# chernistry/sentio

Hardware: NVIDIA H100
Metric: retrieval queries/sec @1M docs,1024-d,top_k=100 (higher is better)
Workload: dtype f16 store / f32 scan / f64 exact re-score

## Files before the change

sentio_b200/csrc/dense_mma.cu:

```cuda
#include <cuda.h>

#include <math.h>

#include <algorithm>
#include <vector>

#include "dense_common.cuh"
#include "dense_mma.cuh"
#include "wgmma.cuh"

namespace {

constexpr int kTileRows = 128;
constexpr int kBK = 64;
constexpr uint32_t kATileBytes = kTileRows * kBK * 2;
constexpr int kConsumerWarps = 8;
constexpr int kMmaThreads = 32 * kConsumerWarps + 32;
constexpr int kQbnMax = 256;
constexpr int kSampleRows = 16;
constexpr int kSampleKeys = kTileRows / kSampleRows;
constexpr int kSelectThreads = 512;
constexpr int kSelStage = 8192;
constexpr int kSelTop = 2048;

__device__ __forceinline__ void tma_load_2d(uint32_t dst, const CUtensorMap* map, int c0, int c1, uint32_t bar,
                                            uint64_t policy) {
  asm volatile(
      "cp.async.bulk.tensor.2d.shared::cluster.global.mbarrier::complete_tx::bytes.L2::cache_hint [%0], [%1, {%2, %3}], "
      "[%4], %5;" ::"r"(dst),
      "l"(map), "r"(c0), "r"(c1), "r"(bar), "l"(policy)
      : "memory");
}
__device__ __forceinline__ void tma_prefetch_l2_2d(const CUtensorMap* map, int c0, int c1) {
  asm volatile("cp.async.bulk.prefetch.tensor.2d.L2.global [%0, {%1, %2}];" ::"l"(map), "r"(c0), "r"(c1) : "memory");
}

struct MmaScanParams {
  const float* inv_norm;
  const float* thr_init;
  unsigned long long* cand;
  int32_t* counts;
  int32_t* fallback;
  int64_t n;
  int32_t kb_count;
  int32_t num_tiles;
  int32_t tile_first, tile_step;
  int32_t capg;
  int32_t stages;
  int32_t prefetch;
  const uint32_t* mask;
  int32_t mask_qs;
  const float* hh;
  const float* rq;
};

template <int QBN, bool FILTER, bool EUCLID>
__global__ void __launch_bounds__(kMmaThreads, 1)
dense_scan_mma_kernel(const __grid_constant__ CUtensorMap tm_rows, const __grid_constant__ CUtensorMap tm_q,
                      const MmaScanParams p) {
  extern __shared__ uint8_t msm_raw[];
  const uint32_t raw = smem_u32(msm_raw);
  const uint32_t base = (raw + 1023u) & ~1023u;
  uint8_t* sm = msm_raw + (base - raw);
  constexpr uint32_t kQBoxBytes = QBN * kBK * 2;
  constexpr uint32_t kStageBytes = kATileBytes + kQBoxBytes;
  uint64_t* bars = reinterpret_cast<uint64_t*>(sm + (size_t)p.stages * kStageBytes);
  const uint32_t bar_full = smem_u32(bars), bar_empty = smem_u32(bars + p.stages);
  volatile float* thr = reinterpret_cast<volatile float*>(bars + 2 * p.stages);
  int* cnt = reinterpret_cast<int*>(const_cast<float*>(thr) + QBN);
  float* rq_s = reinterpret_cast<float*>(cnt + QBN);

  const int warp = threadIdx.x >> 5, lane = threadIdx.x & 31;
  const int grid = gridDim.x, cta = blockIdx.x;
  const int my_tiles = cta < p.num_tiles ? (p.num_tiles - 1 - cta) / grid + 1 : 0;
  auto tile_row = [&](int t) { return (p.tile_first + (cta + t * grid) * p.tile_step) * kTileRows; };

  if (threadIdx.x == 0) {
    for (int s = 0; s < p.stages; ++s) {
      mbar_init(bar_full + 8 * s, 1);
      mbar_init(bar_empty + 8 * s, kConsumerWarps);
    }
    mbar_fence_init();
    asm volatile("prefetch.tensormap [%0];" ::"l"(&tm_rows) : "memory");
    asm volatile("prefetch.tensormap [%0];" ::"l"(&tm_q) : "memory");
  }
  for (int i = threadIdx.x; i < QBN; i += blockDim.x) {
    thr[i] = p.thr_init ? p.thr_init[i] : -INFINITY;
    cnt[i] = 0;
    if constexpr (EUCLID) rq_s[i] = p.rq[i];
  }
  __syncthreads();

  if (warp == kConsumerWarps) {
    if (lane == 0) {
      const uint64_t pol_corpus = policy_evict_first();
      const uint64_t pol_query = policy_evict_last();
      int it = 0;
      const int total_it = my_tiles * p.kb_count;
      for (int t = 0; t < my_tiles; ++t) {
        const int row = tile_row(t);
        for (int kb = 0; kb < p.kb_count; ++kb, ++it) {
          const int s = it % p.stages;
          const uint32_t use = (uint32_t)(it / p.stages);
          const int pf = it + p.stages + p.prefetch;
          if (p.prefetch > 0 && pf < total_it) {
            const int pt = pf / p.kb_count, pkb = pf - pt * p.kb_count;
            tma_prefetch_l2_2d(&tm_rows, pkb * kBK, tile_row(pt));
          }
          if (it >= p.stages) mbar_wait(bar_empty + 8 * s, (use & 1u) ^ 1u);
          const uint32_t stage = base + (uint32_t)s * kStageBytes;
          mbar_expect_tx(bar_full + 8 * s, kStageBytes);
          tma_load_2d(stage, &tm_rows, kb * kBK, row, bar_full + 8 * s, pol_corpus);
          tma_load_2d(stage + kATileBytes, &tm_q, kb * kBK, 0, bar_full + 8 * s, pol_query);
        }
      }
    }
  } else {
    const int wg = warp >> 2;
    unsigned long long* my_cand = p.cand + (size_t)cta * p.capg;
    const size_t q_stride = (size_t)grid * p.capg;
    int it = 0;
    for (int t = 0; t < my_tiles; ++t) {
      float acc[QBN / 2];
      for (int kb = 0; kb < p.kb_count; ++kb, ++it) {
        const int s = it % p.stages;
        mbar_wait(bar_full + 8 * s, (uint32_t)(it / p.stages) & 1u);
        const uint32_t stage = base + (uint32_t)s * kStageBytes;
        const uint64_t da = wgmma_desc_sw128(stage + (uint32_t)wg * (kATileBytes / 2));
        const uint64_t db = wgmma_desc_sw128(stage + kATileBytes);
        wgmma_fence();
#pragma unroll
        for (int k = 0; k < kBK / 16; ++k)
          Wgmma<QBN>::mma(acc, da + (uint64_t)(2 * k), db + (uint64_t)(2 * k), (kb | k) ? 1u : 0u);
        wgmma_commit();
        wgmma_wait<1>();
        __syncwarp();
        if (kb > 0 && lane == 0) mbar_arrive(bar_empty + 8 * ((it - 1) % p.stages));
      }
      wgmma_wait<0>();
      __syncwarp();
      if (lane == 0) mbar_arrive(bar_empty + 8 * ((it - 1) % p.stages));
      const int64_t row0 = (int64_t)tile_row(t) + wg * 64 + (warp & 3) * 16 + (lane >> 2);
      const bool live0 = row0 < p.n, live1 = row0 + 8 < p.n;
      const float invn0 = live0 ? __ldg(p.inv_norm + row0) : 0.f;
      const float invn1 = live1 ? __ldg(p.inv_norm + row0 + 8) : 0.f;
      float h0 = 0.f, h1 = 0.f;
      if constexpr (EUCLID) {
        h0 = live0 ? __ldg(p.hh + row0) : 0.f;
        h1 = live1 ? __ldg(p.hh + row0 + 8) : 0.f;
      }
      auto key = [&](float a, float invn, float h, int col) {
        float s = a * invn;
        if constexpr (EUCLID) s = __fsub_rn(__fmul_rn(rq_s[col], s), h);
        return s;
      };
      const uint32_t* mrow = nullptr;
      if constexpr (FILTER) mrow = p.mask + (size_t)(row0 >> 5) * p.mask_qs + 2 * (lane & 3);
      const int sh0 = (int)(row0 & 31), sh1 = sh0 + 8;
      if (p.thr_init == nullptr) {
        const int slot = t * kSampleKeys + warp;
#pragma unroll
        for (int j = 0; j < QBN / 4; j += 2) {
          uint2 mw = make_uint2(0u, 0u);
          if constexpr (FILTER) mw = __ldg(reinterpret_cast<const uint2*>(mrow + 4 * j));
#pragma unroll
          for (int e = 0; e < 2; ++e) {
            bool m0 = live0, m1 = live1;
            if constexpr (FILTER) {
              const uint32_t w = e ? mw.y : mw.x;
              m0 = m0 && ((w >> sh0) & 1u);
              m1 = m1 && ((w >> sh1) & 1u);
            }
            const int col = 4 * j + 2 * (lane & 3) + e;
            const float s0 = m0 ? key(acc[2 * j + e], invn0, h0, col) : -INFINITY;
            const float s1 = m1 ? key(acc[2 * j + 2 + e], invn1, h1, col) : -INFINITY;
            uint32_t best = max(f32_orderable(s0), f32_orderable(s1));
            best = max(best, __shfl_xor_sync(0xffffffffu, best, 4));
            best = max(best, __shfl_xor_sync(0xffffffffu, best, 8));
            best = max(best, __shfl_xor_sync(0xffffffffu, best, 16));
            if (lane < 4) my_cand[(size_t)col * q_stride + slot] = ((unsigned long long)best << 32) | 0xffffffffull;
          }
        }
      } else {
#pragma unroll
        for (int j = 0; j < QBN / 4; j += 2) {
          uint2 mw = make_uint2(0u, 0u);
          if constexpr (FILTER) mw = __ldg(reinterpret_cast<const uint2*>(mrow + 4 * j));
#pragma unroll
          for (int h = 0; h < 2; ++h) {
            if (!(h ? live1 : live0)) continue;
            const int64_t row = row0 + 8 * h;
            const float invn = h ? invn1 : invn0;
            const float hrow = h ? h1 : h0;
#pragma unroll
            for (int e = 0; e < 2; ++e) {
              const int col = 4 * j + 2 * (lane & 3) + e;
              const float score = key(acc[2 * j + 2 * h + e], invn, hrow, col);
              bool match = true;
              if constexpr (FILTER) match = ((e ? mw.y : mw.x) >> (h ? sh1 : sh0)) & 1u;
              if (score >= thr[col] && match) {
                const int pos = atomicAdd(&cnt[col], 1);
                if (pos < p.capg) my_cand[(size_t)col * q_stride + pos] = make_key32(score, (uint32_t)row);
              }
            }
          }
        }
      }
    }
  }
  __syncthreads();
  for (int i = threadIdx.x; i < QBN; i += blockDim.x) {
    const int c = p.thr_init == nullptr ? my_tiles * kSampleKeys : cnt[i];
    p.counts[(size_t)i * grid + cta] = min(c, p.capg);
    if (c > p.capg && p.fallback) p.fallback[i] = 1;
  }
}

struct SelectParams {
  const unsigned long long* cand;
  const int32_t* counts;
  int32_t grid, capg;
  int32_t nq;
  int32_t mode;
  float* thr_out;
  const float* eps;
  int32_t* fallback;
  const __half* rows;
  const float* q;
  int32_t d_pad, ch;
  int64_t id_base;
  int32_t k;
  int64_t* out_ids;
  double* out_scores;
  int32_t* out_counts;
  const int32_t* state;
  int32_t metric;
  const double* cfac;
  const float* rows32;
};

template <bool FILTER, bool F32>
__global__ void __launch_bounds__(kSelectThreads, 2) dense_select_kernel(const SelectParams p) {
  extern __shared__ __align__(16) uint8_t ssm[];
  unsigned long long* keys = reinterpret_cast<unsigned long long*>(ssm);
  unsigned long long* top = keys + kSelStage;
  unsigned long long* ek = top + kSelTop;
  uint32_t* ei = reinterpret_cast<uint32_t*>(ek + kSelTop);
  __shared__ double qq_s;
  __shared__ int s_prefix[kSelectThreads + 1];
  __shared__ int s_hist[256];
  __shared__ int s_scal[4];
  __shared__ int s_ntop;
  const int tid = threadIdx.x, nt = blockDim.x, lane = tid & 31, warp = tid >> 5, nw = nt >> 5, qi = blockIdx.x;
  const int K = p.k, G = p.grid;
  if (p.mode == 0 && qi >= p.nq) {
    if (tid == 0) p.thr_out[qi] = INFINITY;
    return;
  }
  if constexpr (FILTER) {
    if (p.state[qi]) {
      if (p.mode == 0 && tid == 0) p.thr_out[qi] = INFINITY;
      return;
    }
  }
  if (p.fallback[qi] != 0) {
    if (p.mode == 0 && tid == 0) p.thr_out[qi] = INFINITY;
    return;
  }
  const int32_t* counts = p.counts + (size_t)qi * G;
  const unsigned long long* cand = p.cand + (size_t)qi * G * p.capg;
  {
    const int v = tid < G ? counts[tid] : 0;
    int x = v;
    for (int o = 1; o < 32; o <<= 1) {
      const int y = __shfl_up_sync(0xffffffffu, x, o);
      if (lane >= o) x += y;
    }
    if (lane == 31) s_hist[warp] = x;
    if (tid == 0) s_ntop = 0;
    __syncthreads();
    if (warp == 0) {
      int w = lane < nw ? s_hist[lane] : 0;
      for (int o = 1; o < 32; o <<= 1) {
        const int y = __shfl_up_sync(0xffffffffu, w, o);
        if (lane >= o) w += y;
      }
      s_hist[32 + lane] = w;
    }
    __syncthreads();
    const int incl = x + (warp ? s_hist[32 + warp - 1] : 0);
    if (tid < G) s_prefix[tid] = incl - v;
    if (tid == G - 1) s_prefix[G] = incl;
    __syncthreads();
  }
  const int total = s_prefix[G];
  const bool staged = total <= kSelStage;
  if (staged) {
    for (int g = warp; g < G; g += nw) {
      const int c = s_prefix[g + 1] - s_prefix[g];
      const unsigned long long* src = cand + (size_t)g * p.capg;
      unsigned long long* dst = keys + s_prefix[g];
      for (int i = lane; i < c; i += 32) dst[i] = src[i];
    }
    __syncthreads();
  }
#define SB_FOR_EACH_KEY(BODY)                                                       \
  if (staged) {                                                                     \
    for (int i_ = tid; i_ < total; i_ += nt) {                                      \
      const unsigned long long key = keys[i_];                                      \
      BODY                                                                          \
    }                                                                               \
  } else {                                                                          \
    for (int g_ = warp; g_ < G; g_ += nw) {                                         \
      const int c_ = s_prefix[g_ + 1] - s_prefix[g_];                               \
      const unsigned long long* src_ = cand + (size_t)g_ * p.capg;                  \
      for (int i_ = lane; i_ < c_; i_ += 32) {                                      \
        const unsigned long long key = src_[i_];                                    \
        BODY                                                                        \
      }                                                                             \
    }                                                                               \
  }

  unsigned long long prefix = 0ull, mask = 0ull;
  if (total > K) {
    int need = K;
    for (int shift = 56; shift >= 0; shift -= 8) {
      for (int i = tid; i < 256; i += nt) s_hist[i] = 0;
      __syncthreads();
      SB_FOR_EACH_KEY(if ((key & mask) == prefix) {
        const int dgt = (int)((key >> shift) & 0xffull);
        const unsigned grp = __match_any_sync(__activemask(), dgt);
        if ((int)(threadIdx.x & 31) == __ffs(grp) - 1) atomicAdd(&s_hist[dgt], __popc(grp));
      })
      __syncthreads();
      if (warp == 0) warp_select_bin<true>(s_hist, need, lane, s_scal);
      __syncthreads();
      prefix |= (unsigned long long)s_scal[0] << shift;
      mask |= 0xffull << shift;
      need = s_scal[1];
      const int bucket = s_scal[2];
      __syncthreads();
      if (bucket <= 16) break;
    }
  }
  const float eps = p.eps[qi];
  const unsigned long long lo_key = total > K ? window_lo_key(prefix, eps) : 0ull;
  if (p.mode == 0) {
    if (tid == 0) p.thr_out[qi] = total > K ? key32_score(lo_key) : -INFINITY;
    return;
  }
  SB_FOR_EACH_KEY(if (key >= lo_key) {
    const int at = atomicAdd(&s_ntop, 1);
    if (at < kSelTop) top[at] = key;
  })
#undef SB_FOR_EACH_KEY
  __syncthreads();
  const int ntop = s_ntop;
  if (ntop > kSelTop) {
    if (tid == 0) p.fallback[qi] = 1;
    return;
  }
  int P = 32;
  while (P < ntop) P <<= 1;
  RescoreArgs ra;
  ra.rows = p.rows;
  ra.q = p.q + (size_t)qi * p.d_pad;
  ra.d_pad = p.d_pad;
  ra.ch = p.ch;
  ra.id_base = p.id_base;
  ra.k = p.k;
  ra.out_ids = p.out_ids + (size_t)qi * p.k;
  ra.out_scores = p.out_scores + (size_t)qi * p.k;
  ra.out_count = p.out_counts + qi;
  ra.metric = p.metric;
  ra.cfac = p.cfac;
  ra.rows32 = p.rows32;
  rescore_and_emit<F32>(top, ntop, P, ek, ei, &qq_s, reinterpret_cast<float*>(keys), ra);
}

typedef CUresult (*EncodeTiledFn)(CUtensorMap*, CUtensorMapDataType, cuuint32_t, void*, const cuuint64_t*,
                                  const cuuint64_t*, const cuuint32_t*, const cuuint32_t*, CUtensorMapInterleave,
                                  CUtensorMapSwizzle, CUtensorMapL2promotion, CUtensorMapFloatOOBfill);

int encode_map(CUtensorMap* map, const void* ptr, int64_t rows, int64_t cols, int box_rows) {
  static EncodeTiledFn fn = nullptr;
  if (!fn) {
    void* pfn = nullptr;
    cudaDriverEntryPointQueryResult qres;
    if (cudaGetDriverEntryPoint("cuTensorMapEncodeTiled", &pfn, cudaEnableDefault, &qres) == cudaSuccess &&
        qres == cudaDriverEntryPointSuccess)
      fn = reinterpret_cast<EncodeTiledFn>(pfn);
  }
  SB_REQUIRE(fn != nullptr, SB_ERR_CUDA, "cuTensorMapEncodeTiled entry point not available");
  cuuint64_t dims[2] = {(cuuint64_t)cols, (cuuint64_t)rows};
  cuuint64_t strides[1] = {(cuuint64_t)cols * 2};
  cuuint32_t box[2] = {(cuuint32_t)kBK, (cuuint32_t)box_rows};
  cuuint32_t estr[2] = {1, 1};
  CUresult r = fn(map, CU_TENSOR_MAP_DATA_TYPE_FLOAT16, 2, const_cast<void*>(ptr), dims, strides, box, estr,
                  CU_TENSOR_MAP_INTERLEAVE_NONE, CU_TENSOR_MAP_SWIZZLE_128B, CU_TENSOR_MAP_L2_PROMOTION_L2_256B,
                  CU_TENSOR_MAP_FLOAT_OOB_FILL_NONE);
  SB_REQUIRE(r == CUDA_SUCCESS, SB_ERR_CUDA, "cuTensorMapEncodeTiled failed with CUresult %d", (int)r);
  return SB_OK;
}

size_t mma_per_query(bool euclid) { return euclid ? 12 : 8; }
int mma_stages(const sb_ctx* ctx, int qbn, bool euclid = false) {
  const size_t stage = kATileBytes + (size_t)qbn * kBK * 2 + 16;
  const size_t fixed = 1024 + (size_t)qbn * mma_per_query(euclid);
  return std::min((int)((ctx->smem_optin - fixed) / stage), ctx->dense_max_stages);
}
size_t mma_smem(int qbn, int stages, bool euclid) {
  return 1024 + (size_t)stages * (kATileBytes + (size_t)qbn * kBK * 2 + 16) + (size_t)qbn * mma_per_query(euclid);
}

template <int QBN, bool FILTER, bool EUCLID>
int launch_mma(const CUtensorMap& tm_rows, const CUtensorMap& tm_q, const MmaScanParams& mp, int grid, size_t smem,
               cudaStream_t st) {
  auto kern = dense_scan_mma_kernel<QBN, FILTER, EUCLID>;
  SB_CUDA(cudaFuncSetAttribute(kern, cudaFuncAttributeMaxDynamicSharedMemorySize, (int)smem));
  kern<<<grid, kMmaThreads, smem, st>>>(tm_rows, tm_q, mp);
  SB_CUDA(cudaGetLastError());
  return SB_OK;
}

template <bool FILTER, bool EUCLID>
int dispatch_mma(int qbn, const CUtensorMap& tm_rows, const CUtensorMap& tm_q, const MmaScanParams& mp, int grid,
                 size_t smem, cudaStream_t st) {
  switch (qbn) {
    case 16: return launch_mma<16, FILTER, EUCLID>(tm_rows, tm_q, mp, grid, smem, st);
    case 32: return launch_mma<32, FILTER, EUCLID>(tm_rows, tm_q, mp, grid, smem, st);
    case 64: return launch_mma<64, FILTER, EUCLID>(tm_rows, tm_q, mp, grid, smem, st);
    case 128: return launch_mma<128, FILTER, EUCLID>(tm_rows, tm_q, mp, grid, smem, st);
    case 256: return launch_mma<256, FILTER, EUCLID>(tm_rows, tm_q, mp, grid, smem, st);
  }
  sb_set_error("dense_mma: unsupported query block %d", qbn);
  return SB_ERR_UNSUPPORTED;
}

}

bool dense_mma_eligible(const sb_ctx* ctx, const DenseIndex& ix, int B) {
  if (B < 16) return false;
  if (ix.d_pad % kBK != 0 || ix.n_pad % kTileRows != 0) return false;
  if (ix.n < 64 * kTileRows) return false;
  return mma_stages(ctx, kQbnMax) >= 3;
}

int dense_mma_topk_enqueue(sb_ctx* ctx, DenseIndex& ix, const float* q_pad, int B, int k, int64_t* out_ids,
                           double* out_scores, int32_t* out_counts, cudaStream_t st, const DenseFilter* flt) {
  const int kb_count = ix.d_pad / kBK;
  const int total_tiles = (int)(ix.n_pad / kTileRows);
  const int gsz = kQbnMax;
  const int grid = std::min(ctx->num_sms, total_tiles);
  const double phi = flt ? std::min(1.0, (double)std::max<int64_t>(flt->c_min, 1) / (double)ix.n) : 1.0;
  const double hit = flt ? 1.0 - pow(1.0 - phi, (double)kSampleRows) : 1.0;
  const double m_eff = flt ? (double)kSampleRows * phi / hit : (double)kSampleRows;
  const int per_cta = flt ? std::max(ctx->dense_sample_per_cta,
                                     (int)ceil(4.0 * k / ((double)kSampleKeys * hit * grid)))
                          : std::max(ctx->dense_sample_per_cta, std::min(8, (4 * k / kSampleKeys + grid - 1) / grid));
  const int sample_tiles = (int)std::min<int64_t>((int64_t)per_cta * grid, total_tiles);
  const int sample_step = total_tiles / sample_tiles;
  const int sgrid = std::min(grid, sample_tiles);
  const int64_t worst = (int64_t)((total_tiles + grid - 1) / grid + 1) * kTileRows;
  const int64_t samp_keys = (int64_t)((sample_tiles + sgrid - 1) / sgrid + 1) * kSampleKeys;
  const double f = (double)k / ((double)kSampleKeys * sample_tiles * hit);
  const double pass = f >= 0.95 ? 1.0 : -log(1.0 - f) / m_eff;
  const int64_t expect = (int64_t)((double)worst * phi * pass) + 1;
  const int capg = (int)std::min<int64_t>(worst, std::max<int64_t>(8 * expect + 256, samp_keys));
  int rc;
  SB_REQUIRE(grid <= kSelectThreads, SB_ERR_UNSUPPORTED, "dense_mma: %d CTAs exceed the select kernel's prefix width", grid);
  const int n_groups = (B + gsz - 1) / gsz;
  const size_t cand_per_group = (size_t)gsz * grid * capg * 8;
  int gmax = (int)std::max<size_t>(1, (size_t)(1024ull << 20) / cand_per_group);
  gmax = std::min(gmax, n_groups);
  if ((rc = ctx->misc2_dev.reserve((size_t)n_groups * gsz * ix.d_pad * 2 + 256))) return rc;
  if ((rc = ctx->misc3_dev.reserve(((size_t)gsz * 4 + (size_t)gsz * grid * 4) * gmax + 256))) return rc;
  if ((rc = ctx->cand_dev.reserve(cand_per_group * gmax))) return rc;
  __half* q16 = ctx->misc2_dev.as<__half>();
  float* thr = ctx->misc3_dev.as<float>();
  int32_t* counts = reinterpret_cast<int32_t*>(thr + (size_t)gsz * gmax);
  unsigned long long* cand = ctx->cand_dev.as<unsigned long long>();
  if (ix.tm_rows_ptr != ix.rows || ix.tm_n_pad != ix.n_pad) {
    if ((rc = encode_map(reinterpret_cast<CUtensorMap*>(ix.tm_rows), ix.rows, ix.n_pad, ix.d_pad, kTileRows))) return rc;
    ix.tm_rows_ptr = ix.rows;
    ix.tm_n_pad = ix.n_pad;
  }
  const CUtensorMap& tm_rows = *reinterpret_cast<const CUtensorMap*>(ix.tm_rows);
  const size_t sel_smem = (size_t)kSelStage * 8 + (size_t)kSelTop * 20 + 64;
  const bool f32 = ix.rows32 != nullptr;
  auto sel_kern = flt ? (f32 ? dense_select_kernel<true, true> : dense_select_kernel<true, false>)
                      : (f32 ? dense_select_kernel<false, true> : dense_select_kernel<false, false>);
  SB_CUDA(cudaFuncSetAttribute(sel_kern, cudaFuncAttributeMaxDynamicSharedMemorySize, (int)sel_smem));
  auto launch_select = [&](int nblocks, const SelectParams& s) {
    sel_kern<<<nblocks, kSelectThreads, sel_smem, st>>>(s);
  };
  const bool euclid = ix.metric == SB_METRIC_EUCLID;
  auto run_mma = [&](int qbn, const CUtensorMap& tm_q, const MmaScanParams& m, int g, size_t smem) {
    if (euclid)
      return flt ? dispatch_mma<true, true>(qbn, tm_rows, tm_q, m, g, smem, st)
                 : dispatch_mma<false, true>(qbn, tm_rows, tm_q, m, g, smem, st);
    return flt ? dispatch_mma<true, false>(qbn, tm_rows, tm_q, m, g, smem, st)
               : dispatch_mma<false, false>(qbn, tm_rows, tm_q, m, g, smem, st);
  };
  float *eps = nullptr, *rq = nullptr;
  int32_t* fb = nullptr;
  if ((rc = dense_prep_queries(ctx, ix, q_pad, B, n_groups * gsz, true, nullptr, q16, &eps, &fb, &rq, st)))
    return rc;

  for (int c0 = 0; c0 < B; c0 += gmax * gsz) {
    const int nq_chunk = std::min(B - c0, gmax * gsz);
    const int ng = (nq_chunk + gsz - 1) / gsz;
    struct Group { int qbn, nq; CUtensorMap tm_q; size_t smem; int stages; };
    std::vector<Group> gs((size_t)ng);
    int rows_total = 0;
    for (int g = 0; g < ng; ++g) {
      Group& G = gs[(size_t)g];
      const int left = nq_chunk - g * gsz;
      __half* q16g = q16 + (size_t)(c0 + g * gsz) * ix.d_pad;
      G.qbn = gsz;
      while (G.qbn > 16 && G.qbn / 2 >= left) G.qbn >>= 1;
      G.nq = std::min(G.qbn, left);
      if ((rc = encode_map(&G.tm_q, q16g, G.qbn, ix.d_pad, G.qbn))) return rc;
      G.stages = mma_stages(ctx, G.qbn, euclid);
      G.smem = mma_smem(G.qbn, G.stages, euclid);
      rows_total = g * gsz + G.qbn;
    }
    MmaScanParams mp;
    mp.inv_norm = ix.inv_norm;
    mp.n = ix.n;
    mp.kb_count = kb_count;
    mp.capg = capg;
    mp.prefetch = ctx->dense_prefetch;
    mp.mask_qs = flt ? flt->qs : 0;
    mp.hh = ix.hh;
    SelectParams sp;
    sp.metric = ix.metric;
    sp.cfac = ix.cfac;
    sp.rows32 = ix.rows32;
    sp.cand = cand;
    sp.counts = counts;
    sp.capg = capg;
    sp.nq = nq_chunk;
    sp.thr_out = thr;
    sp.eps = eps + c0;
    sp.fallback = fb + c0;
    sp.rows = ix.rows;
    sp.q = q_pad + (size_t)c0 * ix.d_pad;
    sp.d_pad = ix.d_pad;
    sp.ch = ix.d_pad / 8;
    sp.id_base = ix.id_base;
    sp.k = k;
    sp.out_ids = out_ids + (size_t)c0 * k;
    sp.out_scores = out_scores + (size_t)c0 * k;
    sp.out_counts = out_counts + c0;
    sp.state = flt ? flt->state + c0 : nullptr;
    mp.thr_init = nullptr;
    mp.fallback = nullptr;
    mp.num_tiles = sample_tiles;
    mp.tile_first = 0;
    mp.tile_step = sample_step;
    {
      ProfScope ps(ctx, SB_PROF_DENSE_SAMPLE, st, ng + 1);
      for (int g = 0; g < ng; ++g) {
        const Group& G = gs[(size_t)g];
        mp.cand = cand + (size_t)g * gsz * sgrid * capg;
        mp.counts = counts + (size_t)g * gsz * sgrid;
        mp.stages = G.stages;
        mp.mask = flt ? flt->mask + c0 + (size_t)g * gsz : nullptr;
        mp.rq = rq ? rq + c0 + (size_t)g * gsz : nullptr;
        if ((rc = run_mma(G.qbn, G.tm_q, mp, sgrid, G.smem))) return rc;
      }
      sp.grid = sgrid;
      sp.mode = 0;
      launch_select(rows_total, sp);
    }
    SB_CUDA(cudaGetLastError());
    mp.num_tiles = total_tiles;
    mp.tile_first = 0;
    mp.tile_step = 1;
    for (int g = 0; g < ng; ++g) {
      const Group& G = gs[(size_t)g];
      mp.thr_init = thr + (size_t)g * gsz;
      mp.fallback = fb + c0 + (size_t)g * gsz;
      mp.cand = cand + (size_t)g * gsz * grid * capg;
      mp.counts = counts + (size_t)g * gsz * grid;
      mp.stages = G.stages;
      mp.mask = flt ? flt->mask + c0 + (size_t)g * gsz : nullptr;
      mp.rq = rq ? rq + c0 + (size_t)g * gsz : nullptr;
      ProfScope ps(ctx, SB_PROF_DENSE_SCAN, st);
      if ((rc = run_mma(G.qbn, G.tm_q, mp, grid, G.smem))) return rc;
    }
    sp.grid = grid;
    sp.mode = 1;
    {
      ProfScope ps(ctx, SB_PROF_DENSE_MERGE, st);
      launch_select(nq_chunk, sp);
    }
    SB_CUDA(cudaGetLastError());
  }
  return dense_fallback_enqueue(ctx, ix, q_pad, B, k, fb, out_ids, out_scores, out_counts, st, flt);
}
```

Baseline: 191,300.

## Use three consumer warpgroups with 192-row tiles and register reallocation

Enlarges the corpus tile from 128 to 192 rows, served by three consumer warpgroups plus a full producer warpgroup. setmaxnreg moves registers from the producer to the consumers. The 256-wide query case is split into two 128-wide wgmma calls so the accumulators fit the new register budget. The epilogue now uses a named barrier over the consumer threads only, and mask loads are guarded for dead rows. The change adds tail handling for row counts not divisible by 192, and depends on the TMA box and shared-memory stage sizes matching the new tile height.

```diff
diff --git a/sentio_b200/csrc/dense_mma.cu b/sentio_b200/csrc/dense_mma.cu
--- a/sentio_b200/csrc/dense_mma.cu
+++ b/sentio_b200/csrc/dense_mma.cu
@@ -11,11 +11,13 @@
 
 namespace {
 
-constexpr int kTileRows = 128;
+constexpr int kTileRows = 192;
 constexpr int kBK = 64;
 constexpr uint32_t kATileBytes = kTileRows * kBK * 2;
-constexpr int kConsumerWarps = 8;
-constexpr int kMmaThreads = 32 * kConsumerWarps + 32;
+constexpr uint32_t kWgRowBytes = 64 * kBK * 2;
+constexpr int kConsumerWarps = 12;
+constexpr int kMmaThreads = 32 * kConsumerWarps + 128;
+constexpr int kConsumerRegs = 160, kProducerRegs = 32;
 constexpr int kQbnMax = 256;
 constexpr int kSampleRows = 16;
 constexpr int kSampleKeys = kTileRows / kSampleRows;
@@ -91,8 +93,9 @@
   }
   __syncthreads();
 
-  if (warp == kConsumerWarps) {
-    if (lane == 0) {
+  if (warp >= kConsumerWarps) {
+    asm volatile("setmaxnreg.dec.sync.aligned.u32 %0;" ::"n"(kProducerRegs));
+    if (warp == kConsumerWarps && lane == 0) {
       const uint64_t pol_corpus = policy_evict_first();
       const uint64_t pol_query = policy_evict_last();
       int it = 0;
@@ -116,6 +119,7 @@
       }
     }
   } else {
+    asm volatile("setmaxnreg.inc.sync.aligned.u32 %0;" ::"n"(kConsumerRegs));
     const int wg = warp >> 2;
     unsigned long long* my_cand = p.cand + (size_t)cta * p.capg;
     const size_t q_stride = (size_t)grid * p.capg;
@@ -126,12 +130,20 @@
         const int s = it % p.stages;
         mbar_wait(bar_full + 8 * s, (uint32_t)(it / p.stages) & 1u);
         const uint32_t stage = base + (uint32_t)s * kStageBytes;
-        const uint64_t da = wgmma_desc_sw128(stage + (uint32_t)wg * (kATileBytes / 2));
+        const uint64_t da = wgmma_desc_sw128(stage + (uint32_t)wg * kWgRowBytes);
         const uint64_t db = wgmma_desc_sw128(stage + kATileBytes);
         wgmma_fence();
 #pragma unroll
-        for (int k = 0; k < kBK / 16; ++k)
-          Wgmma<QBN>::mma(acc, da + (uint64_t)(2 * k), db + (uint64_t)(2 * k), (kb | k) ? 1u : 0u);
+        for (int k = 0; k < kBK / 16; ++k) {
+          const uint32_t sc = (kb | k) ? 1u : 0u;
+          if constexpr (QBN == 256) {
+            Wgmma<128>::mma(*reinterpret_cast<float(*)[64]>(acc), da + (uint64_t)(2 * k), db + (uint64_t)(2 * k), sc);
+            Wgmma<128>::mma(*reinterpret_cast<float(*)[64]>(acc + 64), da + (uint64_t)(2 * k),
+                            db + (uint64_t)((128 * kBK * 2) >> 4) + (uint64_t)(2 * k), sc);
+          } else {
+            Wgmma<QBN>::mma(acc, da + (uint64_t)(2 * k), db + (uint64_t)(2 * k), sc);
+          }
+        }
         wgmma_commit();
         wgmma_wait<1>();
         __syncwarp();
@@ -162,7 +174,7 @@
 #pragma unroll
         for (int j = 0; j < QBN / 4; j += 2) {
           uint2 mw = make_uint2(0u, 0u);
-          if constexpr (FILTER) mw = __ldg(reinterpret_cast<const uint2*>(mrow + 4 * j));
+          if constexpr (FILTER) if (live0) mw = __ldg(reinterpret_cast<const uint2*>(mrow + 4 * j));
 #pragma unroll
           for (int e = 0; e < 2; ++e) {
             bool m0 = live0, m1 = live1;
@@ -185,7 +197,7 @@
 #pragma unroll
         for (int j = 0; j < QBN / 4; j += 2) {
           uint2 mw = make_uint2(0u, 0u);
-          if constexpr (FILTER) mw = __ldg(reinterpret_cast<const uint2*>(mrow + 4 * j));
+          if constexpr (FILTER) if (live0) mw = __ldg(reinterpret_cast<const uint2*>(mrow + 4 * j));
 #pragma unroll
           for (int h = 0; h < 2; ++h) {
             if (!(h ? live1 : live0)) continue;
@@ -207,12 +219,12 @@
         }
       }
     }
-  }
-  __syncthreads();
-  for (int i = threadIdx.x; i < QBN; i += blockDim.x) {
-    const int c = p.thr_init == nullptr ? my_tiles * kSampleKeys : cnt[i];
-    p.counts[(size_t)i * grid + cta] = min(c, p.capg);
-    if (c > p.capg && p.fallback) p.fallback[i] = 1;
+    asm volatile("bar.sync 1, %0;" ::"n"(32 * kConsumerWarps) : "memory");
+    for (int i = threadIdx.x; i < QBN; i += 32 * kConsumerWarps) {
+      const int c = p.thr_init == nullptr ? my_tiles * kSampleKeys : cnt[i];
+      p.counts[(size_t)i * grid + cta] = min(c, p.capg);
+      if (c > p.capg && p.fallback) p.fallback[i] = 1;
+    }
   }
 }
 
@@ -441,15 +453,15 @@
 
 bool dense_mma_eligible(const sb_ctx* ctx, const DenseIndex& ix, int B) {
   if (B < 16) return false;
-  if (ix.d_pad % kBK != 0 || ix.n_pad % kTileRows != 0) return false;
-  if (ix.n < 64 * kTileRows) return false;
+  if (ix.d_pad % kBK != 0 || ix.n_pad % 128 != 0) return false;
+  if (ix.n < 8192) return false;
   return mma_stages(ctx, kQbnMax) >= 3;
 }
 
 int dense_mma_topk_enqueue(sb_ctx* ctx, DenseIndex& ix, const float* q_pad, int B, int k, int64_t* out_ids,
                            double* out_scores, int32_t* out_counts, cudaStream_t st, const DenseFilter* flt) {
   const int kb_count = ix.d_pad / kBK;
-  const int total_tiles = (int)(ix.n_pad / kTileRows);
+  const int total_tiles = (int)((ix.n_pad + kTileRows - 1) / kTileRows);
   const int gsz = kQbnMax;
   const int grid = std::min(ctx->num_sms, total_tiles);
   const double phi = flt ? std::min(1.0, (double)std::max<int64_t>(flt->c_min, 1) / (double)ix.n) : 1.0;
```

Result: faster. 203,700, median of 6 (+6.5%).
